# rslmtoasa/rslmtoasa

Measured on AMD Instinct MI355X. Metric: block-recursion throughput (H|psi> + A_n + B_n recursion levels, recursion.f90 recur_b), higher is better.
Workload: dtype f64

## Files before the change

### rslmtoasa_amd/csrc/kernels_spmm5.hpp

```cpp
#pragma once
#include <hip/hip_runtime.h>
#include <algorithm>
#include <type_traits>
#include <vector>
#include "kernels_valu.hpp"
#include "kernels_mfma.hpp"
#include "kernels_spmm4.hpp"

namespace rsrec {

#ifndef RSREC_S5_KSPLIT_PROBE
#define RSREC_S5_KSPLIT_PROBE 0
#endif
#ifndef RSREC_S5_PRIO
#define RSREC_S5_PRIO 0
#endif
#ifndef S5_WG_GROUPS
#define S5_WG_GROUPS 4
#endif
constexpr int S5_TRIPLE = 640;
constexpr int S5_TRIPLE_BYTES = S5_TRIPLE * 8;
constexpr int S5_HEAD_TRIPLES = 2;
constexpr int S5_HEAD_DOUBLES = 2 * S5_HEAD_TRIPLES * S5_TRIPLE;
constexpr int S5_MAXENT = 2 * S4_MAXSLOTS + 2;
constexpr int S5_ENTPAD = 8;

struct S5Desc { const double* a; const double* b; double sign; double diag; };

__device__ __forceinline__ double s5_desc_value(const S5Desc& D, int ro, int ri, int c ) {
    double v = D.sign * D.a[2 * (ro + 18 * ri) + c];
    if (D.b) v = v + D.b[2 * (ro + 18 * ri) + c];
    if (D.diag != 0.0 && ro == ri && c == 0) v = v + D.diag;
    return v;
}

__global__ __launch_bounds__(640) void k_s5_emit(const S5Desc* __restrict__ desc, const int* __restrict__ meta, int meta_stride, int nfs, int null_col, int ntr,
                                                 double* __restrict__ frag) {
    const int t = blockIdx.x, sig = blockIdx.y, st = blockIdx.z;
    const int* codes = meta + (size_t)st * meta_stride + 2;
    const S5Desc* D = desc + (size_t)st * nfs;
    const int e0 = threadIdx.x;
    const int K = e0 < 256 ? 0 : e0 < 512 ? 1 : 2;
    const int r = e0 - (K == 0 ? 0 : K == 1 ? 256 : 512);
    int q, l, e;
    if (K < 2) { q = r >> 7; l = (r & 127) >> 1; e = r & 1; } else { q = r >> 6; l = r & 63; e = 0; }
    const int k = l >> 4, rho = q == 0 ? (l & 15) : 16 + (l & 3);
    const int stq = rho >> 2, ll = rho & 3;
    int po = 0, mo = 0;
    bool row = true;
    if (stq < 4) { po = stq & 1; mo = 4 * (stq >> 1) + ll; } else if (ll < 2) { po = ll; mo = 8; } else row = false;
    const int o0 = 10 * t + (K == 0 ? 0 : K == 1 ? 4 : 8);
    const int o = K < 2 ? o0 + k : o0 + (k >> 1);
    const int pi = K < 2 ? e : (k & 1);
    double v = 0.0;
    if (row) {
        const int j = o / 9, code = codes[j], col = code & 255, flip = code >> 8;
        if (col != null_col && D[col].a) {
            const int so = sig, si = flip ? 1 - sig : sig, mi = o % 9;
            const int ro = 9 * so + mo, ri = 9 * si + mi;
            const double hr = s5_desc_value(D[col], ro, ri, 0), hi = s5_desc_value(D[col], ro, ri, 1);
            v = (po == pi) ? hr : (po == 0 ? -hi : hi);
        }
    }
    frag[(((size_t)st * 2 + sig) * ntr + t) * S5_TRIPLE + e0] = v;
}

struct Spmm5Operator {
    double* d_frag = nullptr;
    int* d_meta = nullptr;
    size_t frag_bytes = 0, meta_bytes = 0;
    S5Desc* d_desc = nullptr;
    size_t desc_bytes = 0;
    std::vector<signed char> sched_sig;
    int sched_dims[3] = {0, 0, 0};
    int sched_epoch = 0;
    int ntau = 0, nslots = 0, have_o = 0, ntr = 0, spin_mixing = 0;
    static constexpr int META = 2 + S5_MAXENT + S5_ENTPAD;
    struct Entry { const double* blk; int col; int flip; };
    struct Head { std::vector<double> blk; int flip = 0; bool valid = false; };
    std::vector<Head> head_main;
    std::vector<int> ksteps;
    std::vector<signed char> mixing;

    Spmm5Operator() = default;
    Spmm5Operator(const Spmm5Operator&) = delete;
    Spmm5Operator& operator=(const Spmm5Operator&) = delete;
    ~Spmm5Operator() { release(); }
    void release() {
        if (d_frag) (void)hipFree(d_frag);
        if (d_meta) (void)hipFree(d_meta);
        if (d_desc) (void)hipFree(d_desc);
        d_frag = nullptr; d_meta = nullptr; d_desc = nullptr; frag_bytes = meta_bytes = desc_bytes = 0;
        sched_sig.clear();
    }
    static bool decode20(int rho, int& part, int& m) {
        const int st = rho >> 2, l = rho & 3;
        if (st < 4) { part = st & 1; m = 4 * (st >> 1) + l; return true; }
        if (l < 2) { part = l; m = 8; return true; }
        return false;
    }
    static double hreal(const double* blk, int so, int po, int mo, int si, int pi, int mi) {
        const int ro = 9 * so + mo, ri = 9 * si + mi;
        const double hr = blk[2 * (ro + 18 * ri)], hi = blk[2 * (ro + 18 * ri) + 1];
        if (po == pi) return hr;
        return po == 0 ? -hi : hi;
    }
    static int steps_of(int nent) {
        const int n = 9 * nent, r = n % 10;
        return 3 * (n / 10) + (r == 0 ? 0 : r <= 4 ? 1 : r <= 8 ? 2 : 3);
    }
// ... 17 lines not shown
                    }
            }
        }
    }
    const char* make_schedule(int nslots_lat, int ntau_, int nset, const std::vector<signed char>& kind, std::vector<std::vector<std::pair<int, int>>>* sched_out) {
        if (nslots_lat + 1 > S4_MAXSLOTS) return "too many neighbour slots for the spmm5 kernel";
        const bool same = !sched_out && d_meta && sched_dims[0] == nslots_lat && sched_dims[1] == ntau_ && sched_dims[2] == nset && sched_sig == kind;
        if (same) return nullptr;
        ++sched_epoch;
        ntau = ntau_; nslots = nslots_lat; have_o = nset > 1 ? 1 : 0; spin_mixing = 0;
        const int nfs = nslots + 1, null_col = nslots + 1;
        std::vector<std::vector<std::pair<int, int>>> sched((size_t)nset * ntau);
        std::vector<int> meta((size_t)nset * ntau * META, 0);
        ksteps.assign((size_t)nset * ntau, 0);
        mixing = kind;
        int maxent = 0;
        for (int set = 0; set < nset; ++set)
            for (int tau = 0; tau < ntau; ++tau) {
                std::vector<std::pair<int, int>>& E = sched[(size_t)set * ntau + tau];
                const signed char* Kd = kind.data() + ((size_t)set * ntau + tau) * nfs;
                int* M = meta.data() + ((size_t)set * ntau + tau) * META;
                if (Kd[nslots] >= 0) {
                    E.push_back({nslots, 0});
                    E.push_back({Kd[nslots] == 1 ? nslots : -1, 1});
                    M[1] = 2;
                }
                for (int s = 0; s < nslots; ++s) {
                    if (Kd[s] < 0) continue;
                    E.push_back({s, 0});
                    if (Kd[s] == 1) { E.push_back({s, 1}); if (s > 0) spin_mixing = 1; }
                }
                M[0] = steps_of((int)E.size());
                ksteps[(size_t)set * ntau + tau] = 5 * (M[0] / 3) + 2 * (M[0] % 3);
                for (int j = 0; j < S5_MAXENT + S5_ENTPAD; ++j)
                    M[2 + j] = j < (int)E.size() ? ((E[j].first >= 0 ? E[j].first : null_col) | (E[j].second << 8)) : null_col;
                maxent = std::max(maxent, (int)E.size());
            }
        ntr = (9 * maxent + 9) / 10 + 1;
        const size_t need = (size_t)nset * ntau * 2 * ntr * S5_TRIPLE * sizeof(double), mneed = meta.size() * sizeof(int);
        if (need > frag_bytes) {
            if (d_frag) (void)hipFree(d_frag);
            d_frag = nullptr; frag_bytes = 0;
            if (hipMalloc(reinterpret_cast<void**>(&d_frag), need) != hipSuccess) return "hipMalloc of spmm5 operator fragments failed";
            frag_bytes = need;
        }
        if (mneed > meta_bytes) {
            if (d_meta) (void)hipFree(d_meta);
            d_meta = nullptr; meta_bytes = 0;
            if (hipMalloc(reinterpret_cast<void**>(&d_meta), mneed) != hipSuccess) return "hipMalloc of spmm5 schedule failed";
            meta_bytes = mneed;
        }
        if (hipMemcpy(d_meta, meta.data(), mneed, hipMemcpyHostToDevice) != hipSuccess) return "upload of spmm5 schedule failed";
        sched_sig = kind; sched_dims[0] = nslots_lat; sched_dims[1] = ntau_; sched_dims[2] = nset;
        if (sched_out) sched_out->swap(sched);
        return nullptr;
    }
    static std::vector<signed char> kinds_of(const std::vector<const double*>& blk) {
        std::vector<signed char> kind(blk.size(), -1);
        for (size_t q = 0; q < blk.size(); ++q)
            if (blk[q]) kind[q] = Spmm4Operator::pattern_of(blk[q]) == 0 ? 1 : 0;
        return kind;
    }
    const char* build_custom(int nslots_lat, int ntau_, int nset, const std::vector<const double*>& blk) {
        std::vector<std::vector<std::pair<int, int>>> sched;
        if (const char* msg = make_schedule(nslots_lat, ntau_, nset, kinds_of(blk), &sched)) return msg;
        const int nfs = nslots + 1;
        head_main.assign((size_t)nset * ntau, Head());
        const size_t per_sig = (size_t)ntr * S5_TRIPLE, per_set = (size_t)ntau * 2 * per_sig;
// ... 105 lines not shown
template <int NL, int NM>
__device__ __forceinline__ void s5_interleave() {
    constexpr int PER = NM / NL;
#pragma unroll
    for (int i = 0; i < NL; ++i) {
        __builtin_amdgcn_sched_group_barrier(0x20, 1, 0);
        __builtin_amdgcn_sched_group_barrier(0x8, PER, 0);
    }
    __builtin_amdgcn_sched_group_barrier(0x8, NM - PER * NL, 0);
}

template <int NL = 11>
__device__ __forceinline__ void s5_mfma(S5Acc& acc, const S5Pair& o) {
#pragma unroll
    for (int e = 0; e < 2; ++e)
#pragma unroll
        for (int t = 0; t < 9; ++t) {
            acc.m[t] = __builtin_amdgcn_mfma_f64_16x16x4f64(o.a[0][e], o.b[t][e], acc.m[t], 0, 0, 0);
            acc.r[t] = __builtin_amdgcn_mfma_f64_4x4x4f64(o.a[1][e], o.b[t][e], acc.r[t], 0, 0, 0);
        }
    s5_interleave<NL, 36>();
}
template <int NL = 11>
__device__ __forceinline__ void s5_mfma(S5Acc& acc, const S5Single& o) {
#pragma unroll
    for (int t = 0; t < 9; ++t) {
        acc.m[t] = __builtin_amdgcn_mfma_f64_16x16x4f64(o.a[0], o.b[t], acc.m[t], 0, 0, 0);
        acc.r[t] = __builtin_amdgcn_mfma_f64_4x4x4f64(o.a[1], o.b[t], acc.r[t], 0, 0, 0);
    }
    s5_interleave<NL, 18>();
}

template <int N> using S5C = std::integral_constant<int, N>;
#define S5_GLOBAL __attribute__((address_space(1)))
#define S5_CONST __attribute__((address_space(4)))
#define S5_LDS __attribute__((address_space(3)))
typedef const S5_GLOBAL char* s5_gp;

template <bool TWO, bool LDSA, bool OCT = false>
__device__ __forceinline__ void s5_run_stream(S5Acc& acc, const int* __restrict__ meta, const char* __restrict__ fr , const char* __restrict__ fr_head,
                                              const char* __restrict__ inb, const char* __restrict__ in2b,
                                              const int* __restrict__ nbr5 ,
                                              const int (&atom)[GROUP] , int rem_sel ,
                                              int ncol, int sig, int l4,
                                              unsigned lane_main, unsigned lane_z, unsigned lane_rem, unsigned lane_rem_z, unsigned lane16, unsigned lane8,
                                              const int (&tile_blk)[GROUP], int rem_blk , int kpart = 0) {
    int left = meta[0];
    int ebase = 0, tbase = 0;
    bool first = true;
#if RSREC_S5_KSPLIT_PROBE
    if (kpart == 0) left = min(left, 27);
    else { left -= 27; ebase = 10; tbase = 9; first = false; }
#endif
    if (left <= 0) return;
    const bool extras = TWO && meta[1] != 0;
    const S5_CONST int* codes = (const S5_CONST int*)(meta + 2);
    const S5_CONST int* nbr = (const S5_CONST int*)nbr5;
    S5Ent E0, E1;
    int raw[GROUP];
    int code_cur = codes[ebase], code_nxt = codes[ebase + 1];
    auto load_idx = [&](int col) {
#pragma unroll
        for (int t = 0; t < GROUP; ++t) raw[t] = nbr[(size_t)ncol * atom[t] + col];
    };
    load_idx(code_cur & 255);
    unsigned vlane_main = lane_main, vlane_z = lane_z, vlane16 = lane16, vlane8 = lane8;
    auto open_entry = [&](int j, S5Ent& E) {
        const unsigned so = 2592u * (unsigned)((code_cur >> 8) ? 1 - sig : sig);
#pragma unroll
        for (int t = 0; t < GROUP; ++t) E.off[t] = (unsigned)(OCT ? raw[t] + tile_blk[t] : raw[t]) * (BLD * 8u) + so;
        const int r01 = (rem_sel & 1) ? raw[1] : raw[0], r23 = (rem_sel & 1) ? raw[3] : raw[2], r45 = (rem_sel & 1) ? raw[5] : raw[4], r67 = (rem_sel & 1) ? raw[7] : raw[6];
        const int r03 = (rem_sel & 2) ? r23 : r01, r47 = (rem_sel & 2) ? r67 : r45;
        E.rem = (unsigned)(((rem_sel & 4) ? r47 : r03) + (OCT ? rem_blk : 0)) * (BLD * 8u) + so;
        code_cur = code_nxt;
        code_nxt = codes[j + 2];
        load_idx(code_cur & 255);
    };
    auto issue = [&](auto s2c, auto& o) {
        constexpr int S2 = decltype(s2c)::value, S = S2 % 27, wrap = S2 / 27;
        using I = S5St<S>;
        S5Ent& EA = (I::eA & 1) ? E1 : E0;
        S5Ent& EB = (I::eA & 1) ? E0 : E1;
        if constexpr (I::opens) open_entry(ebase + 10 * wrap + I::eOpen, (I::eOpen & 1) ? E1 : E0);
        const bool head = wrap == 0 && first && extras;
        const char* __restrict__ base = (TWO && S < 5 && head) ? in2b : inb;
        s5_gp fbg = nullptr;
        if constexpr (!LDSA) {
            const char* fb = ((TWO && I::T < S5_HEAD_TRIPLES && head && fr_head) ? fr_head + I::T * S5_TRIPLE_BYTES
                                                                                 : fr + (size_t)(tbase + 9 * wrap + I::T) * S5_TRIPLE_BYTES)
// ... 31 lines not shown
#pragma unroll
            for (int q = 0; q < 2; ++q) o.a[q] = *(const S5_LDS V*)(fl + lf + q * (I::K < 2 ? 1024 : 512));
        } else if constexpr (I::K < 2) {
#pragma unroll
            for (int q = 0; q < 2; ++q) o.a[q] = *(const S5_GLOBAL V*)(fbg + lf + q * 1024);
        } else {
#pragma unroll
            for (int q = 0; q < 2; ++q) o.a[q] = *(const S5_GLOBAL V*)(fbg + lf + q * 512);
        }
    };
    S5Pair X, Y;
    S5Single Z;
    issue(S5C<0>{}, X);
    issue(S5C<1>{}, Y);
#define S5_STEP(S, NEXT, CUR)                 \
    if (left > (S)) {                         \
        issue(S5C<(S) + 2>{}, NEXT);          \
        s5_mfma<LDSA ? 9 : 11>(acc, CUR);     \
        __builtin_amdgcn_sched_barrier(0);    \
    }
    for (;; left -= 27) {
        S5_STEP(0, Z, X) S5_STEP(1, X, Y) S5_STEP(2, Y, Z) S5_STEP(3, Z, X) S5_STEP(4, X, Y) S5_STEP(5, Y, Z)
        S5_STEP(6, Z, X) S5_STEP(7, X, Y) S5_STEP(8, Y, Z) S5_STEP(9, Z, X) S5_STEP(10, X, Y) S5_STEP(11, Y, Z)
        S5_STEP(12, Z, X) S5_STEP(13, X, Y) S5_STEP(14, Y, Z) S5_STEP(15, Z, X) S5_STEP(16, X, Y) S5_STEP(17, Y, Z)
        S5_STEP(18, Z, X) S5_STEP(19, X, Y) S5_STEP(20, Y, Z) S5_STEP(21, Z, X) S5_STEP(22, X, Y) S5_STEP(23, Y, Z)
        S5_STEP(24, Z, X) S5_STEP(25, X, Y) S5_STEP(26, Y, Z)
        if (left <= 27) break;
        ebase += 10; tbase += 9; first = false;
    }
#undef S5_STEP
}


template <int NT> struct S5PairN { s5_d2 b[NT]; s5_d2 a[2]; };
template <int NT> struct S5SingleN { double b[NT]; double a[2]; };
template <int NT> struct S5AccN { double4_t m[NT]; double r[NT]; };

template <int NT>
__device__ __forceinline__ void s5_mfma_n(S5AccN<NT>& acc, const S5PairN<NT>& o) {
#pragma unroll
    for (int e = 0; e < 2; ++e)
#pragma unroll
        for (int t = 0; t < NT; ++t) {
            acc.m[t] = __builtin_amdgcn_mfma_f64_16x16x4f64(o.a[0][e], o.b[t][e], acc.m[t], 0, 0, 0);
            acc.r[t] = __builtin_amdgcn_mfma_f64_4x4x4f64(o.a[1][e], o.b[t][e], acc.r[t], 0, 0, 0);
        }
    s5_interleave<NT, 4 * NT>();
}
template <int NT>
__device__ __forceinline__ void s5_mfma_n(S5AccN<NT>& acc, const S5SingleN<NT>& o) {
#pragma unroll
    for (int t = 0; t < NT; ++t) {
        acc.m[t] = __builtin_amdgcn_mfma_f64_16x16x4f64(o.a[0], o.b[t], acc.m[t], 0, 0, 0);
        acc.r[t] = __builtin_amdgcn_mfma_f64_4x4x4f64(o.a[1], o.b[t], acc.r[t], 0, 0, 0);
    }
    s5_interleave<NT, 2 * NT>();
}

struct S5EntN { unsigned off[3]; unsigned rem; };

template <bool TWO, int NMAIN, bool HASREM>
__device__ __forceinline__ void s5_run_stream_n(S5AccN<NMAIN + (HASREM ? 1 : 0)>& acc, const int* __restrict__ meta, const char* __restrict__ fr ,
                                                const char* __restrict__ inb, const char* __restrict__ in2b, const int* __restrict__ nbr5,
                                                const int (&atom)[NMAIN], const int (&ratom)[GROUP], int rem_sel, int ncol, int sig, int l4,
                                                unsigned lane_main, unsigned lane_z, unsigned lane_rem, unsigned lane_rem_z, unsigned lane16, unsigned lane8) {
    constexpr int NT = NMAIN + (HASREM ? 1 : 0);
// ... 68 lines not shown
        const S5_LDS char* fl = (const S5_LDS char*)fr + (unsigned)(tbase + 9 * wrap + I::T) * S5_TRIPLE_BYTES + (I::K == 0 ? 0 : I::K == 1 ? 2048 : 4096);
#pragma unroll
        for (int q = 0; q < 2; ++q) o.a[q] = *(const S5_LDS V*)(fl + lf + q * (I::K < 2 ? 1024 : 512));
    };
    S5PairN<NT> X0, Y0, X1, Y1;
    S5SingleN<NT> Z0, Z1;
    issue(S5C<0>{}, X0);
    issue(S5C<1>{}, Y0);
    issue(S5C<2>{}, Z0);
    issue(S5C<3>{}, X1);
    issue(S5C<4>{}, Y1);
#define S5_STEP(S, NEXT, CUR)                 \
    if (left > (S)) {                         \
        issue(S5C<(S) + 5>{}, NEXT);          \
        s5_mfma_n<NT>(acc, CUR);              \
        __builtin_amdgcn_sched_barrier(0);    \
    }
    for (;; left -= 54) {
        S5_STEP(0, Z1, X0) S5_STEP(1, X0, Y0) S5_STEP(2, Y0, Z0) S5_STEP(3, Z0, X1) S5_STEP(4, X1, Y1) S5_STEP(5, Y1, Z1)
        S5_STEP(6, Z1, X0) S5_STEP(7, X0, Y0) S5_STEP(8, Y0, Z0) S5_STEP(9, Z0, X1) S5_STEP(10, X1, Y1) S5_STEP(11, Y1, Z1)
        S5_STEP(12, Z1, X0) S5_STEP(13, X0, Y0) S5_STEP(14, Y0, Z0) S5_STEP(15, Z0, X1) S5_STEP(16, X1, Y1) S5_STEP(17, Y1, Z1)
        S5_STEP(18, Z1, X0) S5_STEP(19, X0, Y0) S5_STEP(20, Y0, Z0) S5_STEP(21, Z0, X1) S5_STEP(22, X1, Y1) S5_STEP(23, Y1, Z1)
        S5_STEP(24, Z1, X0) S5_STEP(25, X0, Y0) S5_STEP(26, Y0, Z0) S5_STEP(27, Z0, X1) S5_STEP(28, X1, Y1) S5_STEP(29, Y1, Z1)
        S5_STEP(30, Z1, X0) S5_STEP(31, X0, Y0) S5_STEP(32, Y0, Z0) S5_STEP(33, Z0, X1) S5_STEP(34, X1, Y1) S5_STEP(35, Y1, Z1)
        S5_STEP(36, Z1, X0) S5_STEP(37, X0, Y0) S5_STEP(38, Y0, Z0) S5_STEP(39, Z0, X1) S5_STEP(40, X1, Y1) S5_STEP(41, Y1, Z1)
        S5_STEP(42, Z1, X0) S5_STEP(43, X0, Y0) S5_STEP(44, Y0, Z0) S5_STEP(45, Z0, X1) S5_STEP(46, X1, Y1) S5_STEP(47, Y1, Z1)
        S5_STEP(48, Z1, X0) S5_STEP(49, X0, Y0) S5_STEP(50, Y0, Z0) S5_STEP(51, Z0, X1) S5_STEP(52, X1, Y1) S5_STEP(53, Y1, Z1)
        if (left <= 54) break;
        ebase += 20; tbase += 18; first = false;
    }
#undef S5_STEP
}

struct S5Epilogue { int kind = 0; const double* cur = nullptr; const double* old = nullptr; double a = 1.0, b = 0.0; };

struct S5Gram { double* out = nullptr; size_t cstride = 0; long min_groups = 0; };

template <bool TWO, bool LDSA, bool OCT = false, int NSP = 1, bool GRAM = false>
__global__ __launch_bounds__(NSP == 3 ? 768 : S5_WG_GROUPS * 128) void k_spmm5(SpmmDims D, const int* __restrict__ order_all, const int* __restrict__ cum,
                                               const int* __restrict__ nbr ,
                                               const int* __restrict__ izp, const double* __restrict__ frag, const int* __restrict__ meta, int ntr,
                                               const double* __restrict__ in_all, double* __restrict__ out_all,
                                               const double* __restrict__ in2_all = nullptr,
                                               const double* __restrict__ frag_head = nullptr ,
                                               int ntau = 0, int lds_tau = 0 ,
                                               int* __restrict__ queue = nullptr ,
                                               int spin_by_xcd = 1 ,
                                               S5Epilogue epi = S5Epilogue(), S5Gram gram = S5Gram()) {
    static_assert(!GRAM || (!TWO && !OCT && NSP == 1), "the Gram epilogue: one input, whole groups of atoms");
    extern __shared__ double s5_lds[];
    const int lane = threadIdx.x & 63;
    const int wave = __builtin_amdgcn_readfirstlane(threadIdx.x >> 6);
    const int sig = LDSA ? (int)((spin_by_xcd ? blockIdx.x : (blockIdx.x >> 3)) & 1) : wave / S5_WG_GROUPS, gslot = LDSA ? wave : wave % S5_WG_GROUPS;
#if RSREC_S5_PRIO
    if (wave >= (int)(blockDim.x >> 7)) __builtin_amdgcn_s_setprio(1);
#endif
    const int WGG = LDSA ? (int)(blockDim.x >> 6) : S5_WG_GROUPS;
    int bxl = blockIdx.x, gdxl = gridDim.x, run_lo = D.run_lo, run_hi = D.run_hi, qrun = 0;
    if (LDSA && D.nruns > 0) {
        const int row = spin_by_xcd ? 8 : 16, rowi = (int)blockIdx.x / row;
        int r = 0;
#pragma unroll
        for (int q = 1; q < 4; ++q) if (q < D.nruns && rowi >= D.run_row0[q]) r = q;
        lds_tau = D.run_tau[r]; run_lo = D.run_glo[r]; run_hi = D.run_ghi[r];
        bxl = (int)blockIdx.x - row * D.run_row0[r];
        gdxl = row * (D.run_row0[r + 1] - D.run_row0[r]);
        qrun = r;
    }
    if constexpr (LDSA) {
        const s5_d2* __restrict__ src = reinterpret_cast<const s5_d2*>(frag + ((size_t)lds_tau * 2 + sig) * ntr * S5_TRIPLE);
        s5_d2* dst = reinterpret_cast<s5_d2*>(s5_lds);
        const int n = ntr * (S5_TRIPLE / 2);
        constexpr int PER = (int)(160 * 1024 / 16 / (NSP == 3 ? 512 : S5_WG_GROUPS * 64));
        const int nthr = (int)blockDim.x;
        s5_d2 v[PER];
#pragma unroll
        for (int i = 0; i < PER; ++i) { const int e = threadIdx.x + i * nthr; if (e < n) v[i] = src[e]; }
#pragma unroll
        for (int i = 0; i < PER; ++i) { const int e = threadIdx.x + i * nthr; if (e < n) dst[e] = v[i]; }
        __syncthreads();
    }
    const int l15 = lane & 15, l4 = lane >> 4;
    const unsigned lane_main = 8u * (36 * l4 + 2 * l15), lane_z = 8u * (36 * (l4 >> 1) + 2 * l15 + (l4 & 1));
    const unsigned lane_rem = 8u * (36 * l4 + 32 + 2 * (l15 & 1)), lane_rem_z = 8u * (36 * (l4 >> 1) + 32 + 2 * (l15 & 1) + (l4 & 1));
    const unsigned lane16 = 16u * lane, lane8 = 8u * lane;
    const int ncol = D.nslots + 2;
#pragma unroll 1
    for (int chain = OCT ? GROUP * (int)blockIdx.y : (int)blockIdx.y; chain < D.nchains; chain += OCT ? GROUP * (int)gridDim.y : (int)gridDim.y) {
    const int count = cum[(chain / D.cpo) * D.nlev + D.level];
    int ngroups = count / GROUP;
    const bool fold = GRAM && gram.out != nullptr && epi.kind == 0 && s5_gram_folds(ngroups, gram.min_groups);
    const int ob = D.obase[(chain / D.cpo) * D.nlev + D.level];
    const int* __restrict__ order = order_all + (size_t)(chain / D.cpo) * D.ostride + ob;
    const bool on_full_list = D.sat_base > 0 && ob == D.sat_base;
    if constexpr (OCT) ngroups = D.nmax;
    else if (run_hi > 0) {
        if (!on_full_list) continue;
        order += (size_t)run_lo * GROUP;
        ngroups = run_hi - run_lo;
    }
    const bool skipping = D.nskip > 0 && on_full_list;
    const size_t vo = (size_t)chain * D.vstride;
    const char* __restrict__ inb = reinterpret_cast<const char*>(in_all + vo);
    const char* __restrict__ in2b = TWO ? reinterpret_cast<const char*>(in2_all + vo) : nullptr;
    double* __restrict__ out = out_all + vo;
    const int zero_block = D.kk;

    int g, gend, gstep, glo = 0;
    bool dynamic = false;
    {
        const int bx = bxl;
        const int need = (ngroups + WGG - 1) / WGG;
        if constexpr (!LDSA) {
            const int nbx = max(1, min((int)gridDim.x, need));
            if (bx >= nbx) continue;
            if (nbx < 8) { g = bx * WGG + gslot; gend = ngroups; gstep = nbx * WGG; }
            else {
                const int xcd = bx & 7, j = bx >> 3;
                const int per_xcd = (nbx >> 3) + ((xcd < (nbx & 7)) ? 1 : 0);
                const int chunk = (ngroups + 7) >> 3;
                const int lo = xcd * chunk;
                gend = min(ngroups, lo + chunk);
                g = lo + j * WGG + gslot;
                gstep = per_xcd * WGG;
// ... 127 lines not shown
        int atom[GROUP];
        int vatom[GROUP], tile_blk[GROUP];
        int my_rem_atom, rem_blk = 0;
        if constexpr (OCT) {
            const int a0 = g;
#pragma unroll
            for (int t = 0; t < GROUP; ++t) {
                const bool ok = a0 >= 0 && chain + t < D.nchains;
                atom[t] = ok ? a0 : zero_block;
                tile_blk[t] = ok ? t * (D.kk + 1) : 0;
                vatom[t] = ok ? a0 + t * (D.kk + 1) : zero_block;
            }
            const int tr = l15 >> 1;
            const bool okr = a0 >= 0 && chain + tr < D.nchains;
            rem_blk = okr ? tr * (D.kk + 1) : 0;
            my_rem_atom = okr ? a0 + tr * (D.kk + 1) : zero_block;
        } else {
#pragma unroll
            for (int t = 0; t < GROUP; ++t) { const int a = grp[t]; atom[t] = a >= 0 ? a : zero_block; vatom[t] = atom[t]; tile_blk[t] = 0; }
            my_rem_atom = grp[l15 >> 1];
            my_rem_atom = my_rem_atom >= 0 ? my_rem_atom : zero_block;
        }
        const int first = atom[0];
        if (!OCT && D.skip_pa && first < D.nmax) continue;
        const int tau = first < D.nmax ? first : D.nmax + izp[first];
        const int* __restrict__ M = meta + (size_t)tau * Spmm5Operator::META;
        const char* __restrict__ fr = LDSA ? reinterpret_cast<const char*>(s5_lds) : reinterpret_cast<const char*>(frag + ((size_t)tau * 2 + sig) * ntr * S5_TRIPLE);
        const char* __restrict__ fh = (TWO && frag_head) ? reinterpret_cast<const char*>(frag_head + ((size_t)chain * ntau + tau) * S5_HEAD_DOUBLES + (size_t)sig * S5_HEAD_TRIPLES * S5_TRIPLE) : nullptr;

        S5Acc acc;
#pragma unroll
        for (int t = 0; t < 9; ++t) { acc.m[t] = (double4_t){0, 0, 0, 0}; acc.r[t] = 0.0; }

        if constexpr (OCT) s5_run_stream<TWO, LDSA, true>(acc, M, fr, fh, inb, in2b, nbr, atom, l15 >> 1, ncol, sig, l4, lane_main, lane_z, lane_rem, lane_rem_z, lane16, lane8, tile_blk, rem_blk);
        else s5_run_stream<TWO, LDSA>(acc, M, fr, fh, inb, in2b, nbr, atom, l15 >> 1, ncol, sig, l4, lane_main, lane_z, lane_rem, lane_rem_z, lane16, lane8, tile_blk, rem_blk, kpart);
#if RSREC_S5_KSPLIT_PROBE
        if (kpart) continue;
#endif

        if constexpr (GRAM) if (fold) {
            unsigned gl;
            asm volatile("v_mbcnt_lo_u32_b32 %0, -1, 0\n\tv_mbcnt_hi_u32_b32 %0, -1, %0" : "=v"(gl));
            const int lane = (int)gl, l15 = lane & 15, l4 = lane >> 4;
            const double* __restrict__ ub = in_all + vo;
            double4_t gre = {0, 0, 0, 0}, gim = {0, 0, 0, 0};
            double sre[2] = {0.0, 0.0}, sim[2] = {0.0, 0.0}, kre[2] = {0.0, 0.0}, kim[2] = {0.0, 0.0};
            auto rem_coef = [&](s5_d2 u, double& cr, double& ci) {
                cr = l4 == 0 ? u[0] : (l4 == 1 ? u[1] : 0.0);
                ci = l4 == 0 ? -u[1] : (l4 == 1 ? u[0] : 0.0);
            };
            auto gram_tiles = [&](auto t0c, auto t1c) {
                constexpr int T0 = decltype(t0c)::value, T1 = decltype(t1c)::value, NT = T1 - T0;
                s5_d2 gu[NT][3], gs[NT][3][2];
#pragma unroll
                for (int i = 0; i < NT; ++i) {
                    const int t = T0 + i;
                    const double* ab = ub + (size_t)BLD * ((t < 8) ? vatom[t] : my_rem_atom) + 324 * sig;
#pragma unroll
                    for (int p = 0; p < 3; ++p) {
                        const int row = 36 * (p < 2 ? 4 * p + l4 : 8);
                        if (t < 8) gu[i][p] = *reinterpret_cast<const s5_d2*>(ab + row + 2 * l15);
#pragma unroll
                        for (int e = 0; e < 2; ++e) gs[i][p][e] = *reinterpret_cast<const s5_d2*>(ab + row + 32 + 2 * e);
                    }
                }
#pragma unroll
                for (int i = 0; i < NT; ++i) {
                    const int t = T0 + i;
                    const double x8 = acc.r[t];
                    if (t < 8) {
#pragma unroll
                        for (int p = 0; p < 2; ++p) {
                            gre = __builtin_amdgcn_mfma_f64_16x16x4f64(gu[i][p][0], acc.m[t][2 * p], gre, 0, 0, 0);
                            gre = __builtin_amdgcn_mfma_f64_16x16x4f64(gu[i][p][1], acc.m[t][2 * p + 1], gre, 0, 0, 0);
                            gim = __builtin_amdgcn_mfma_f64_16x16x4f64(-gu[i][p][1], acc.m[t][2 * p], gim, 0, 0, 0);
                            gim = __builtin_amdgcn_mfma_f64_16x16x4f64(gu[i][p][0], acc.m[t][2 * p + 1], gim, 0, 0, 0);
                        }
                        double cr, ci;
                        rem_coef(gu[i][2], cr, ci);
                        gre = __builtin_amdgcn_mfma_f64_16x16x4f64(cr, x8, gre, 0, 0, 0);
                        gim = __builtin_amdgcn_mfma_f64_16x16x4f64(ci, x8, gim, 0, 0, 0);
                    }
                    double (&are)[2] = (t < 8) ? sre : kre;
                    double (&aim)[2] = (t < 8) ? sim : kim;
#pragma unroll
                    for (int e = 0; e < 2; ++e) {
#pragma unroll
                        for (int p = 0; p < 2; ++p) {
                            const double ur = gs[i][p][e][0], ui = gs[i][p][e][1], tr = acc.m[t][2 * p], ti = acc.m[t][2 * p + 1];
                            are[e] = fma(ur, tr, are[e]); are[e] = fma(ui, ti, are[e]);
                            aim[e] = fma(ur, ti, aim[e]); aim[e] = fma(-ui, tr, aim[e]);
                        }
                        double cr, ci;
                        rem_coef(gs[i][2][e], cr, ci);
                        are[e] = fma(cr, x8, are[e]);
                        aim[e] = fma(ci, x8, aim[e]);
                    }
                }
            };
            gram_tiles(S5C<0>{}, S5C<2>{});
            __builtin_amdgcn_sched_barrier(0);
            gram_tiles(S5C<2>{}, S5C<4>{});
            __builtin_amdgcn_sched_barrier(0);
            gram_tiles(S5C<4>{}, S5C<6>{});
            __builtin_amdgcn_sched_barrier(0);
            gram_tiles(S5C<6>{}, S5C<8>{});
            __builtin_amdgcn_sched_barrier(0);
            gram_tiles(S5C<8>{}, S5C<9>{});
            __builtin_amdgcn_sched_barrier(0);
            auto sum_l4 = [&](double v) {
                double s = __shfl(v, l15);
                s += __shfl(v, l15 + 16); s += __shfl(v, l15 + 32); s += __shfl(v, l15 + 48);
                return s;
            };
            auto sum_atoms = [&](double v) {
                double s = __shfl(v, l15 & 1);
#pragma unroll
                for (int a = 1; a < GROUP; ++a) s += __shfl(v, 2 * a + (l15 & 1));
                return s;
            };
            double* gp = gram.out + (size_t)chain * gram.cstride + ((size_t)g * 2 + sig) * S5_GRAM_DOUBLES;
            s5_d2 v;
#pragma unroll
            for (int p = 0; p < 2; ++p) {
                v[0] = gre[2 * p]; v[1] = gre[2 * p + 1];
                *reinterpret_cast<s5_d2*>(gp + 4 * lane + 2 * p) = v;
                v[0] = gim[2 * p]; v[1] = gim[2 * p + 1];
                *reinterpret_cast<s5_d2*>(gp + 256 + 4 * lane + 2 * p) = v;
            }
#pragma unroll
            for (int e = 0; e < 2; ++e) {
                v[0] = sum_l4(sre[e]); v[1] = sum_l4(sim[e]);
                if (l4 == e) *reinterpret_cast<s5_d2*>(gp + 512 + 2 * (16 * e + l15)) = v;
                v[0] = sum_atoms(sum_l4(kre[e])); v[1] = sum_atoms(sum_l4(kim[e]));
                if (lane < 2) *reinterpret_cast<s5_d2*>(gp + 576 + 2 * (2 * e + lane)) = v;
            }
        }
        const int ekind = GRAM ? 0 : epi.kind;
        auto finish = [&](auto t0c, auto t1c) {
            constexpr int T0 = decltype(t0c)::value, T1 = decltype(t1c)::value, NT = T1 - T0;
            size_t eo[NT];
#pragma unroll
// ... 12 lines not shown
                    const double* zb = epi.old + vo;
#pragma unroll
                    for (int i = 0; i < NT; ++i) {
#pragma unroll
                        for (int p = 0; p < 2; ++p) ez[i][p] = *reinterpret_cast<const s5_d2*>(zb + eo[i] + 36 * (4 * p + l4));
                        ezr[i] = zb[eo[i] + 288 + (l4 & 1)];
                    }
                }
            }
#pragma unroll
            for (int i = 0; i < NT; ++i) {
                const int t = T0 + i;
                const int a = (t < 8) ? vatom[t] : my_rem_atom;
                double* ob = out + eo[i];
#pragma unroll
                for (int p = 0; p < 2; ++p) {
                    s5_d2 v; v[0] = acc.m[t][2 * p]; v[1] = acc.m[t][2 * p + 1];
                    if (ekind) {
                        v[0] = (v[0] - epi.b * ec[i][p][0]) / epi.a; v[1] = (v[1] - epi.b * ec[i][p][1]) / epi.a;
                        if (ekind == 2) { v[0] = v[0] * 2.0 - ez[i][p][0]; v[1] = v[1] * 2.0 - ez[i][p][1]; }
                    }
                    if (a != zero_block) *reinterpret_cast<s5_d2*>(ob + 36 * (4 * p + l4)) = v;
                }
                double r = acc.r[t];
                if (ekind) {
                    r = (r - epi.b * ecr[i]) / epi.a;
                    if (ekind == 2) r = r * 2.0 - ezr[i];
                }
                if (a != zero_block && l4 < 2) ob[288 + l4] = r;
            }
        };
        finish(S5C<0>{}, S5C<5>{});
        finish(S5C<5>{}, S5C<9>{});
    }
    }
}

}
```

### rslmtoasa_amd/csrc/rsrec.hip

```cpp
#include <hip/hip_runtime.h>
#include <hsa/hsa.h>
#include <hsa/hsa_ext_amd.h>
#include <dlfcn.h>
#include <algorithm>
#include <array>
#include <atomic>
#include <chrono>
#include <cmath>
#include <cstdarg>
#include <cstdio>
#include <cstdlib>
#include <cstring>
#include <memory>
#include <string>
#include <thread>
#include <tuple>
#include <vector>

#include "../../include/rsrec.h"
#include "kernels_valu.hpp"
#include "kernels_mfma.hpp"
#include "kernels_spmm4.hpp"
#include "kernels_spmm5.hpp"
#include "kernels_uscheme.hpp"
// ... 77 lines not shown
    DevBuf d_la_extra, d_rot;
    Spmm5Operator kubo_op[RSREC_KUBO_NOUT_MAX], kubo_op_b[RSREC_KUBO_NIN_MAX], kubo_hbulk;
    Spmm5Operator orb_plain;
    DevBuf d_green_in, d_green_out;
    DevBuf d_kubo[5];
    DevBuf d_cond[4];
    DevBuf d_ctens[2];
    DevBuf d_bsqrt, d_term, d_gim, d_ldos;
    DevBuf d_ops, d_spec;
    struct SpecImage { int nop = 0, nen = 0, n = 0, site_offset = 0, nsites_total = 0; } spec_res;
    DevBuf d_mint;
    void* pin = nullptr;
    size_t pin_bytes = 0;
    DevBuf d_frags, d_vec[6], d_partial, d_partial2, d_coefA, d_coefB, d_bmats, d_status, d_seed, d_seedcoef, d_mu, d_scal, d_zsqr;
    DevBuf d_fan, d_fan_tab, d_mpair;
    DevBuf d_bloch_geo, d_bloch_tab;
    long opt_batch = 0, opt_kernels = 0, opt_nblk = 0, opt_spmm5 = 2, opt_chain_fold = 1, opt_s5_cap = 0, opt_side = 1, opt_s5_lds = 1, opt_s5_queue = 1, opt_cheb_fused = 1;
    long opt_s5_waves = 8;
    long opt_sat_pct = 100;
    long opt_orth_oop = 1;
    long opt_s5_split = 0;
    long opt_s5_run_min = 0;
    long opt_s5_spin_xcd = 0;
    long opt_s5_octet = 8;
    long opt_s5_host_emit = 0;
    long opt_kubo_lchunk = 0;
    long opt_kubo_vbatch = 0;
    long opt_kubo_setgroup = 0;
    int n_kubo_left_chunks = 0;
    int kubo_diag_nvec = 0, kubo_diag_ll = 0;
    long opt_orth3 = 1;
    long opt_graph = 1;
    long opt_s5_gram_min = 256;
    int ham_hermitian = 0;
    std::vector<int> opp_slot;
    int opp_epoch = -1;
    DevBuf d_gram;
    double n_gram_folded = 0, n_gram_all = 0, n_gram_levels = 0;
    hipGraphExec_t graph_exec = nullptr;
    std::vector<uintptr_t> graph_key;
    bool capturing = false;
    double t_total_ms = 0, t_hop_ms = 0, t_rest_ms = 0, t_host_ms = 0;
    double t_rot_ms = 0;
    double n_hop_launch = 0, n_atom_steps = 0, n_block_mult = 0, n_hop_mfma_flop = 0;
    double n_req_flop = 0;
    int hop_fuses_a = 1;
    std::vector<hipEvent_t> ev_pool;
    size_t ev_used = 0;
    struct RegionEntry {
        std::vector<int> seeds;
        int nlev, napply, flags, epoch, ostride;
        double atom_steps, block_mults;
        DevBuf order, cum;
        std::vector<int> level_max;
        std::vector<int> hop_min, hop_max;
        std::vector<double> level_groups;
        std::vector<double> mult_hist;
        struct ClassRun { int tau, lo, hi; };
        std::vector<ClassRun> sat_runs;
        std::vector<int> level_sat;
        int sat_base = 0;
    };
    std::vector<std::unique_ptr<RegionEntry>> region_cache;
    int lattice_epoch = 0;
    const int* cur_order = nullptr;
    const int* cur_cum = nullptr;
// ... 9 lines not shown
    int comm_rank = 0, comm_nranks = 1;
    DevBuf d_comm;
    ~rsrec_handle();
};

namespace {

struct OptionEntry { const char* name; long rsrec_handle::*member; };
const OptionEntry OPTIONS[] = {
    {"batch", &rsrec_handle::opt_batch},
    {"kernels", &rsrec_handle::opt_kernels},
    {"nblk", &rsrec_handle::opt_nblk},
    {"spmm5", &rsrec_handle::opt_spmm5},
    {"chain_fold", &rsrec_handle::opt_chain_fold},
    {"s5_cap", &rsrec_handle::opt_s5_cap},
    {"s5_lds", &rsrec_handle::opt_s5_lds},
    {"s5_queue", &rsrec_handle::opt_s5_queue},
    {"cheb_fused", &rsrec_handle::opt_cheb_fused},
    {"side_stream", &rsrec_handle::opt_side},
    {"graph", &rsrec_handle::opt_graph},
    {"orth3", &rsrec_handle::opt_orth3},
    {"s5_waves", &rsrec_handle::opt_s5_waves},
    {"s5_split", &rsrec_handle::opt_s5_split},
    {"orth_oop", &rsrec_handle::opt_orth_oop},
    {"sat_pct", &rsrec_handle::opt_sat_pct},
    {"kubo_lchunk", &rsrec_handle::opt_kubo_lchunk},
    {"kubo_vbatch", &rsrec_handle::opt_kubo_vbatch},
    {"kubo_setgroup", &rsrec_handle::opt_kubo_setgroup},
    {"s5_host_emit", &rsrec_handle::opt_s5_host_emit},
    {"s5_octet", &rsrec_handle::opt_s5_octet},
    {"s5_spin_xcd", &rsrec_handle::opt_s5_spin_xcd},
    {"s5_run_min", &rsrec_handle::opt_s5_run_min},
    {"s5_gram_min", &rsrec_handle::opt_s5_gram_min},
};

int fail(rsrec_t* h, int code, const char* fmt, ...) {
    char buf[512];
    va_list ap;
    va_start(ap, fmt);
    vsnprintf(buf, sizeof buf, fmt, ap);
    va_end(ap);
    if (h) h->err = buf;
    return code;
}

#define HIPCK(h, call)                                                                                         \
    do {                                                                                                       \
        hipError_t e_ = (call);                                                                                \
        if (e_ != hipSuccess) return fail(h, RSREC_ERR_DEVICE, "%s failed: %s (%s:%d)", #call, hipGetErrorString(e_), __FILE__, __LINE__); \
    } while (0)

hipEvent_t next_event(rsrec_t* h) {
    static const bool off = getenv("RSREC_NO_EVENTS") != nullptr;
    if (off || h->capturing) return nullptr;
    if (h->ev_used == h->ev_pool.size()) {
        hipEvent_t e;
        if (hipEventCreate(&e) != hipSuccess) return nullptr;
        h->ev_pool.push_back(e);
    }
    hipEvent_t e = h->ev_pool[h->ev_used++];
    (void)hipEventRecord(e, h->stream);
    return e;
}

constexpr size_t PIN_BYTES = (size_t)8 << 20;
int pin_ready(rsrec_t* h) {
// ... 847 lines not shown
        dim3 g2(std::max(row, (grid.x + row - 1) / row * row), grid.y);
        int* queue = nullptr;
        const unsigned ncu = (unsigned)std::max(16, h->n_cu / 16 * 16);
        if ((h->opt_s5_queue == 1 && grid.x >= ncu) || h->opt_s5_queue >= 2) {
            if ((!h->capturing || h->d_s5queue.bytes >= (size_t)SD.nchains * 16 * sizeof(int)) &&
                h->d_s5queue.reserve((size_t)SD.nchains * 16 * sizeof(int)) == hipSuccess &&
                hipMemsetAsync(h->d_s5queue.p, 0, (size_t)SD.nchains * 16 * sizeof(int), h->stream) == hipSuccess) {
                queue = h->d_s5queue.as<int>();
                g2 = dim3(ncu, 1);
            }
        }
        const unsigned thr = (queue && h->opt_s5_waves == 4) ? S5_WG_GROUPS * 64 : S5_WG_GROUPS * 128;
        if (queue && h->opt_s5_split == 3) {
            const unsigned thr3 = 64u * (unsigned)std::min<long>(12, std::max<long>(8, h->opt_s5_waves));
            const size_t lds3 = std::min(lds_limit, lds_bytes + (size_t)S5_TRIPLE_BYTES);
            k_spmm5<TWO, true, false, 3><<<g2, thr3, lds3, h->stream>>>(SD, order, cum, h->d_nbr5.as<int>(), iz, op.frag_set(set), op.meta_set(set), op.ntr, in, out, in2, nullptr, ntau, one, queue, spin_by_xcd, epi);
        } else if constexpr (!TWO) {
            if (gram.out) k_spmm5<false, true, false, 1, true><<<g2, thr, lds_bytes, h->stream>>>(SD, order, cum, h->d_nbr5.as<int>(), iz, op.frag_set(set), op.meta_set(set), op.ntr, in, out, in2, nullptr, ntau, one, queue, spin_by_xcd, epi, gram);
            else k_spmm5<false, true><<<g2, thr, lds_bytes, h->stream>>>(SD, order, cum, h->d_nbr5.as<int>(), iz, op.frag_set(set), op.meta_set(set), op.ntr, in, out, in2, nullptr, ntau, one, queue, spin_by_xcd, epi);
        } else
        k_spmm5<TWO, true><<<g2, thr, lds_bytes, h->stream>>>(SD, order, cum, h->d_nbr5.as<int>(), iz, op.frag_set(set), op.meta_set(set), op.ntr, in, out, in2, nullptr, ntau, one, queue, spin_by_xcd, epi);
    } else if constexpr (!TWO) {
        if (gram.out) k_spmm5<false, false, false, 1, true><<<grid, S5_WG_GROUPS * 128, 0, h->stream>>>(SD, order, cum, h->d_nbr5.as<int>(), iz, op.frag_set(set), op.meta_set(set), op.ntr, in, out, in2, extra, ntau, 0, nullptr, 1, epi, gram);
        else k_spmm5<false, false><<<grid, S5_WG_GROUPS * 128, 0, h->stream>>>(SD, order, cum, h->d_nbr5.as<int>(), iz, op.frag_set(set), op.meta_set(set), op.ntr, in, out, in2, extra, ntau, 0, nullptr, 1, epi);
    } else
        k_spmm5<TWO, false><<<grid, S5_WG_GROUPS * 128, 0, h->stream>>>(SD, order, cum, h->d_nbr5.as<int>(), iz, op.frag_set(set), op.meta_set(set), op.ntr, in, out, in2, extra, ntau, 0, nullptr, 1, epi);
}

template <bool TWO>
void launch_s5(rsrec_t* h, dim3 grid, const SpmmDims& SD0, const int* order, const int* cum, const int* iz, const Spmm5Operator& op, int set,
               const double* in, double* out, const double* in2 = nullptr, const double* extra = nullptr, int ntau = 0, S5Epilogue epi = S5Epilogue(),
               S5Gram gram = S5Gram() ) {
    SpmmDims SD = SD0;
    const int one = op.single_class(set);
    const rsrec_handle::RegionEntry* E = h->cur_entry;
    const bool multi = one < 0 && h->opt_s5_lds >= 2 && !extra && E && E->sat_base > 0 && SD.cpo == 1 && SD.level >= 0 && SD.level < (int)E->level_sat.size() &&
                       E->level_sat[SD.level] > 0 && op.ntau == h->nmax + h->ntype && (grid.x >= (unsigned)std::max(16, h->n_cu / 16 * 16) || h->opt_s5_queue >= 2) && (size_t)op.ntr * S5_TRIPLE * sizeof(double) <= (s5_prepare(h), h->s5_lds_limit);
    bool octets = false, oct_aside = false;
    double pa_pairs = 0.0;
    if (h->cur_level_groups && SD.level >= 0 && (size_t)(SD.level + 1) * op.ntau <= h->cur_level_groups->size() && op.ntau == h->nmax + h->ntype)
        for (int t = 0; t < h->nmax; ++t) pa_pairs += (*h->cur_level_groups)[(size_t)SD.level * op.ntau + t];
    if (!multi && one < 0 && h->opt_s5_octet > 0 && h->nmax >= h->opt_s5_octet && !extra && E && SD.cpo == 1 && SD.nchains >= 2 && op.ntau == h->nmax + h->ntype &&
        2.0 * pa_pairs >= (double)h->nmax * SD.nchains && (double)GROUP * (double)(h->kk + 1) * BLD * 8.0 < 4294967296.0) {
        SpmmDims SO = SD;
        const dim3 go((unsigned)((h->nmax + S5_WG_GROUPS - 1) / S5_WG_GROUPS), (unsigned)((SD.nchains + GROUP - 1) / GROUP));
        hipStream_t so = h->stream;
        if (h->opt_side && !h->oct_stream && !h->capturing &&
            (hipStreamCreateWithFlags(&h->oct_stream, hipStreamNonBlocking) != hipSuccess || hipEventCreateWithFlags(&h->ev_oct_in, hipEventDisableTiming) != hipSuccess ||
             hipEventCreateWithFlags(&h->ev_oct_out, hipEventDisableTiming) != hipSuccess)) { h->oct_stream = nullptr; (void)hipGetLastError(); }
        if (h->opt_side && h->oct_stream && h->ev_oct_in && h->ev_oct_out && hipEventRecord(h->ev_oct_in, h->stream) == hipSuccess &&
            hipStreamWaitEvent(h->oct_stream, h->ev_oct_in, 0) == hipSuccess) { so = h->oct_stream; oct_aside = true; }
        k_spmm5<TWO, false, true><<<go, S5_WG_GROUPS * 128, 0, so>>>(SO, order, cum, h->d_nbr5.as<int>(), iz, op.frag_set(set), op.meta_set(set), op.ntr, in, out, in2, nullptr, ntau,
                                                                   0, nullptr, 1, epi);
        if (oct_aside) (void)hipEventRecord(h->ev_oct_out, h->oct_stream);
        const bool all_sat = E->sat_base > 0 && SD.level < (int)E->level_sat.size() && E->level_sat[SD.level] == SD.nchains && (int)E->sat_runs.size() >= h->nmax &&
                             E->sat_runs[0].tau == 0 && E->sat_runs[0].lo == 0 && E->sat_runs[h->nmax - 1].tau == h->nmax - 1 && E->sat_runs[h->nmax - 1].hi == h->nmax;
        if (all_sat) {
            SD.sat_base = E->sat_base; SD.run_lo = h->nmax; SD.run_hi = E->sat_runs.back().hi;
        } else SD.skip_pa = 1;
        octets = true;
        h->n_octet_launch++;
    }
    if (!multi) {
        launch_s5_one<TWO>(h, grid, SD, order, cum, iz, op, set, in, out, in2, extra, ntau, epi, one, gram);
        if (oct_aside) (void)hipStreamWaitEvent(h->stream, h->ev_oct_out, 0);
    } else {
// ... 2849 lines not shown
```

Before: 67190.

## Share Gram remainder strips via DPP broadcasts and add optional self-tail prefetch

The Gram epilogue now loads only its own remainder-row strip once per lane and uses DPP row-broadcast and pair-swap to hand each tile's strip values to the other lanes, replacing the per-tile global loads of those strips. The tiles are processed one at a time with a scheduling barrier after each. An opt-in mode (s5_tail_self, off by default) adds a second code table whose padding points at the self slot and issues touch loads on the remainder atom to warm the cache. The DPP path adds cross-lane moves and more register pressure from keeping all group tiles' gu values live.

```diff
diff --git a/rslmtoasa_amd/csrc/kernels_spmm5.hpp b/rslmtoasa_amd/csrc/kernels_spmm5.hpp
--- a/rslmtoasa_amd/csrc/kernels_spmm5.hpp
+++ b/rslmtoasa_amd/csrc/kernels_spmm5.hpp
@@ -24,6 +24,7 @@
 constexpr int S5_HEAD_DOUBLES = 2 * S5_HEAD_TRIPLES * S5_TRIPLE;
 constexpr int S5_MAXENT = 2 * S4_MAXSLOTS + 2;
 constexpr int S5_ENTPAD = 8;
+constexpr int S5_CODES = S5_MAXENT + S5_ENTPAD;
 
 struct S5Desc { const double* a; const double* b; double sign; double diag; };
 
@@ -75,7 +76,7 @@
     int sched_dims[3] = {0, 0, 0};
     int sched_epoch = 0;
     int ntau = 0, nslots = 0, have_o = 0, ntr = 0, spin_mixing = 0;
-    static constexpr int META = 2 + S5_MAXENT + S5_ENTPAD;
+    static constexpr int META = 2 + 2 * S5_CODES;
     struct Entry { const double* blk; int col; int flip; };
     struct Head { std::vector<double> blk; int flip = 0; bool valid = false; };
     std::vector<Head> head_main;
@@ -159,8 +160,11 @@
                 }
                 M[0] = steps_of((int)E.size());
                 ksteps[(size_t)set * ntau + tau] = 5 * (M[0] / 3) + 2 * (M[0] % 3);
-                for (int j = 0; j < S5_MAXENT + S5_ENTPAD; ++j)
-                    M[2 + j] = j < (int)E.size() ? ((E[j].first >= 0 ? E[j].first : null_col) | (E[j].second << 8)) : null_col;
+                for (int j = 0; j < S5_CODES; ++j) {
+                    const bool real = j < (int)E.size();
+                    M[2 + j] = real ? ((E[j].first >= 0 ? E[j].first : null_col) | (E[j].second << 8)) : null_col;
+                    M[2 + S5_CODES + j] = real ? M[2 + j] : nslots;
+                }
                 maxent = std::max(maxent, (int)E.size());
             }
         ntr = (9 * maxent + 9) / 10 + 1;
@@ -332,6 +336,18 @@
 }
 
 template <int N> using S5C = std::integral_constant<int, N>;
+template <int N>
+__device__ __forceinline__ double s5_row_bcast(double v) {
+    const int lo = __builtin_amdgcn_mov_dpp(__double2loint(v), 0x150 + N, 0xf, 0xf, false);
+    const int hi = __builtin_amdgcn_mov_dpp(__double2hiint(v), 0x150 + N, 0xf, 0xf, false);
+    return __hiloint2double(hi, lo);
+}
+__device__ __forceinline__ double s5_pair_swap(double v) {
+    const int lo = __builtin_amdgcn_mov_dpp(__double2loint(v), 0xB1, 0xf, 0xf, false);
+    const int hi = __builtin_amdgcn_mov_dpp(__double2hiint(v), 0xB1, 0xf, 0xf, false);
+    return __hiloint2double(hi, lo);
+}
+
 #define S5_GLOBAL __attribute__((address_space(1)))
 #define S5_CONST __attribute__((address_space(4)))
 #define S5_LDS __attribute__((address_space(3)))
@@ -344,7 +360,8 @@
                                               const int (&atom)[GROUP] , int rem_sel ,
                                               int ncol, int sig, int l4,
                                               unsigned lane_main, unsigned lane_z, unsigned lane_rem, unsigned lane_rem_z, unsigned lane16, unsigned lane8,
-                                              const int (&tile_blk)[GROUP], int rem_blk , int kpart = 0) {
+                                              const int (&tile_blk)[GROUP], int rem_blk , int kpart = 0,
+                                              bool tail_self = false ) {
     int left = meta[0];
     int ebase = 0, tbase = 0;
     bool first = true;
@@ -354,7 +371,7 @@
 #endif
     if (left <= 0) return;
     const bool extras = TWO && meta[1] != 0;
-    const S5_CONST int* codes = (const S5_CONST int*)(meta + 2);
+    const S5_CONST int* codes = (const S5_CONST int*)(meta + 2 + (tail_self ? S5_CODES : 0));
     const S5_CONST int* nbr = (const S5_CONST int*)nbr5;
     S5Ent E0, E1;
     int raw[GROUP];
@@ -452,6 +469,16 @@
 }
 
 
+__device__ __forceinline__ int s5_touch_tail(const double* __restrict__ ub, int rem_atom, int sig) {
+    unsigned gl;
+    asm volatile("v_mbcnt_lo_u32_b32 %0, -1, 0\n\tv_mbcnt_hi_u32_b32 %0, -1, %0" : "=v"(gl));
+    const int q = (int)(gl & 7);
+    const int blk = __shfl(rem_atom, (int)(gl >> 3) * 2);
+    const unsigned off = q < 7 ? 1728u + 128u * (unsigned)q : 2588u;
+    return *reinterpret_cast<const int*>(reinterpret_cast<const char*>(ub + (size_t)BLD * blk + 324 * sig) + off);
+}
+__device__ __forceinline__ void s5_touch_done(int v) { asm volatile("" ::"v"(v)); }
+
 template <int NT> struct S5PairN { s5_d2 b[NT]; s5_d2 a[2]; };
 template <int NT> struct S5SingleN { double b[NT]; double a[2]; };
 template <int NT> struct S5AccN { double4_t m[NT]; double r[NT]; };
@@ -586,7 +613,7 @@
 #undef S5_STEP
 }
 
-struct S5Epilogue { int kind = 0; const double* cur = nullptr; const double* old = nullptr; double a = 1.0, b = 0.0; };
+struct S5Epilogue { int kind = 0; const double* cur = nullptr; const double* old = nullptr; double a = 1.0, b = 0.0; int tail_self = 0; };
 
 struct S5Gram { double* out = nullptr; size_t cstride = 0; long min_groups = 0; };
 
@@ -644,6 +671,7 @@
     const int count = cum[(chain / D.cpo) * D.nlev + D.level];
     int ngroups = count / GROUP;
     const bool fold = GRAM && gram.out != nullptr && epi.kind == 0 && s5_gram_folds(ngroups, gram.min_groups);
+    const bool tail = epi.tail_self != 0 && (fold || (!GRAM && epi.kind != 0 && epi.cur == in_all));
     const int ob = D.obase[(chain / D.cpo) * D.nlev + D.level];
     const int* __restrict__ order = order_all + (size_t)(chain / D.cpo) * D.ostride + ob;
     const bool on_full_list = D.sat_base > 0 && ob == D.sat_base;
@@ -837,8 +865,10 @@
 #pragma unroll
         for (int t = 0; t < 9; ++t) { acc.m[t] = (double4_t){0, 0, 0, 0}; acc.r[t] = 0.0; }
 
-        if constexpr (OCT) s5_run_stream<TWO, LDSA, true>(acc, M, fr, fh, inb, in2b, nbr, atom, l15 >> 1, ncol, sig, l4, lane_main, lane_z, lane_rem, lane_rem_z, lane16, lane8, tile_blk, rem_blk);
-        else s5_run_stream<TWO, LDSA>(acc, M, fr, fh, inb, in2b, nbr, atom, l15 >> 1, ncol, sig, l4, lane_main, lane_z, lane_rem, lane_rem_z, lane16, lane8, tile_blk, rem_blk, kpart);
+        if constexpr (OCT) s5_run_stream<TWO, LDSA, true>(acc, M, fr, fh, inb, in2b, nbr, atom, l15 >> 1, ncol, sig, l4, lane_main, lane_z, lane_rem, lane_rem_z, lane16, lane8, tile_blk, rem_blk, 0, tail);
+        else s5_run_stream<TWO, LDSA>(acc, M, fr, fh, inb, in2b, nbr, atom, l15 >> 1, ncol, sig, l4, lane_main, lane_z, lane_rem, lane_rem_z, lane16, lane8, tile_blk, rem_blk, kpart, tail);
+        int touched = 0;
+        if constexpr (GRAM) if (tail) touched = s5_touch_tail(in_all + vo, my_rem_atom, sig);
 #if RSREC_S5_KSPLIT_PROBE
         if (kpart) continue;
 #endif
@@ -854,65 +884,72 @@
                 cr = l4 == 0 ? u[0] : (l4 == 1 ? u[1] : 0.0);
                 ci = l4 == 0 ? -u[1] : (l4 == 1 ? u[0] : 0.0);
             };
-            auto gram_tiles = [&](auto t0c, auto t1c) {
-                constexpr int T0 = decltype(t0c)::value, T1 = decltype(t1c)::value, NT = T1 - T0;
-                s5_d2 gu[NT][3], gs[NT][3][2];
-#pragma unroll
-                for (int i = 0; i < NT; ++i) {
-                    const int t = T0 + i;
-                    const double* ab = ub + (size_t)BLD * ((t < 8) ? vatom[t] : my_rem_atom) + 324 * sig;
-#pragma unroll
-                    for (int p = 0; p < 3; ++p) {
-                        const int row = 36 * (p < 2 ? 4 * p + l4 : 8);
-                        if (t < 8) gu[i][p] = *reinterpret_cast<const s5_d2*>(ab + row + 2 * l15);
-#pragma unroll
-                        for (int e = 0; e < 2; ++e) gs[i][p][e] = *reinterpret_cast<const s5_d2*>(ab + row + 32 + 2 * e);
+            s5_d2 rs[3], gu[GROUP][3];
+            {
+                const double* rb = ub + (size_t)BLD * my_rem_atom + 324 * sig + 32 + 2 * (l15 & 1);
+#pragma unroll
+                for (int p = 0; p < 3; ++p) rs[p] = *reinterpret_cast<const s5_d2*>(rb + 36 * (p < 2 ? 4 * p + l4 : 8));
+            }
+#pragma unroll
+            for (int t = 0; t < GROUP; ++t) {
+                const double* ab = ub + (size_t)BLD * vatom[t] + 324 * sig + 2 * l15;
+#pragma unroll
+                for (int p = 0; p < 3; ++p) gu[t][p] = *reinterpret_cast<const s5_d2*>(ab + 36 * (p < 2 ? 4 * p + l4 : 8));
+            }
+            const bool odd = (l15 & 1) != 0;
+            auto strip = [&](auto tc, auto ec, auto pc) {
+                constexpr int t = decltype(tc)::value, e = decltype(ec)::value, p = decltype(pc)::value;
+                s5_d2 g;
+                if constexpr (t < 8) { g[0] = s5_row_bcast<2 * t + e>(rs[p][0]); g[1] = s5_row_bcast<2 * t + e>(rs[p][1]); }
+                else {
+                    const double o0 = s5_pair_swap(rs[p][0]), o1 = s5_pair_swap(rs[p][1]);
+                    g[0] = odd == (e != 0) ? rs[p][0] : o0; g[1] = odd == (e != 0) ? rs[p][1] : o1;
+                }
+                return g;
+            };
+            auto gram_tile = [&](auto tc) {
+                constexpr int t = decltype(tc)::value;
+                const double x8 = acc.r[t];
+                if constexpr (t < 8) {
+#pragma unroll
+                    for (int p = 0; p < 2; ++p) {
+                        gre = __builtin_amdgcn_mfma_f64_16x16x4f64(gu[t][p][0], acc.m[t][2 * p], gre, 0, 0, 0);
+                        gre = __builtin_amdgcn_mfma_f64_16x16x4f64(gu[t][p][1], acc.m[t][2 * p + 1], gre, 0, 0, 0);
+                        gim = __builtin_amdgcn_mfma_f64_16x16x4f64(-gu[t][p][1], acc.m[t][2 * p], gim, 0, 0, 0);
+                        gim = __builtin_amdgcn_mfma_f64_16x16x4f64(gu[t][p][0], acc.m[t][2 * p + 1], gim, 0, 0, 0);
                     }
-                }
-#pragma unroll
-                for (int i = 0; i < NT; ++i) {
-                    const int t = T0 + i;
-                    const double x8 = acc.r[t];
-                    if (t < 8) {
-#pragma unroll
-                        for (int p = 0; p < 2; ++p) {
-                            gre = __builtin_amdgcn_mfma_f64_16x16x4f64(gu[i][p][0], acc.m[t][2 * p], gre, 0, 0, 0);
-                            gre = __builtin_amdgcn_mfma_f64_16x16x4f64(gu[i][p][1], acc.m[t][2 * p + 1], gre, 0, 0, 0);
-                            gim = __builtin_amdgcn_mfma_f64_16x16x4f64(-gu[i][p][1], acc.m[t][2 * p], gim, 0, 0, 0);
-                            gim = __builtin_amdgcn_mfma_f64_16x16x4f64(gu[i][p][0], acc.m[t][2 * p + 1], gim, 0, 0, 0);
-                        }
-                        double cr, ci;
-                        rem_coef(gu[i][2], cr, ci);
-                        gre = __builtin_amdgcn_mfma_f64_16x16x4f64(cr, x8, gre, 0, 0, 0);
-                        gim = __builtin_amdgcn_mfma_f64_16x16x4f64(ci, x8, gim, 0, 0, 0);
-                    }
-                    double (&are)[2] = (t < 8) ? sre : kre;
-                    double (&aim)[2] = (t < 8) ? sim : kim;
-#pragma unroll
-                    for (int e = 0; e < 2; ++e) {
-#pragma unroll
-                        for (int p = 0; p < 2; ++p) {
-                            const double ur = gs[i][p][e][0], ui = gs[i][p][e][1], tr = acc.m[t][2 * p], ti = acc.m[t][2 * p + 1];
-                            are[e] = fma(ur, tr, are[e]); are[e] = fma(ui, ti, are[e]);
-                            aim[e] = fma(ur, ti, aim[e]); aim[e] = fma(-ui, tr, aim[e]);
-                        }
-                        double cr, ci;
-                        rem_coef(gs[i][2][e], cr, ci);
-                        are[e] = fma(cr, x8, are[e]);
-                        aim[e] = fma(ci, x8, aim[e]);
-                    }
-                }
+                    double cr, ci;
+                    rem_coef(gu[t][2], cr, ci);
+                    gre = __builtin_amdgcn_mfma_f64_16x16x4f64(cr, x8, gre, 0, 0, 0);
+                    gim = __builtin_amdgcn_mfma_f64_16x16x4f64(ci, x8, gim, 0, 0, 0);
+                }
+                double (&are)[2] = (t < 8) ? sre : kre;
+                double (&aim)[2] = (t < 8) ? sim : kim;
+                auto column = [&](auto ec) {
+                    constexpr int e = decltype(ec)::value;
+                    auto kstep = [&](auto pc) {
+                        constexpr int p = decltype(pc)::value;
+                        const s5_d2 g = strip(tc, ec, pc);
+                        const double ur = g[0], ui = g[1], tr = acc.m[t][2 * p], ti = acc.m[t][2 * p + 1];
+                        are[e] = fma(ur, tr, are[e]); are[e] = fma(ui, ti, are[e]);
+                        aim[e] = fma(ur, ti, aim[e]); aim[e] = fma(-ui, tr, aim[e]);
+                    };
+                    kstep(S5C<0>{});
+                    kstep(S5C<1>{});
+                    double cr, ci;
+                    rem_coef(strip(tc, ec, S5C<2>{}), cr, ci);
+                    are[e] = fma(cr, x8, are[e]);
+                    aim[e] = fma(ci, x8, aim[e]);
+                };
+                column(S5C<0>{});
+                column(S5C<1>{});
+                __builtin_amdgcn_sched_barrier(0);
             };
-            gram_tiles(S5C<0>{}, S5C<2>{});
-            __builtin_amdgcn_sched_barrier(0);
-            gram_tiles(S5C<2>{}, S5C<4>{});
-            __builtin_amdgcn_sched_barrier(0);
-            gram_tiles(S5C<4>{}, S5C<6>{});
-            __builtin_amdgcn_sched_barrier(0);
-            gram_tiles(S5C<6>{}, S5C<8>{});
-            __builtin_amdgcn_sched_barrier(0);
-            gram_tiles(S5C<8>{}, S5C<9>{});
-            __builtin_amdgcn_sched_barrier(0);
+            gram_tile(S5C<0>{}); gram_tile(S5C<1>{}); gram_tile(S5C<2>{}); gram_tile(S5C<3>{});
+            gram_tile(S5C<4>{}); gram_tile(S5C<5>{}); gram_tile(S5C<6>{}); gram_tile(S5C<7>{});
+            gram_tile(S5C<8>{});
+#pragma unroll
+            for (int e = 0; e < 2; ++e) { asm volatile("" : "+v"(sre[e]), "+v"(sim[e]), "+v"(kre[e]), "+v"(kim[e])); }
             auto sum_l4 = [&](double v) {
                 double s = __shfl(v, l15);
                 s += __shfl(v, l15 + 16); s += __shfl(v, l15 + 32); s += __shfl(v, l15 + 48);
@@ -991,8 +1028,9 @@
         };
         finish(S5C<0>{}, S5C<5>{});
         finish(S5C<5>{}, S5C<9>{});
-    }
-    }
-}
-
-}
+        if constexpr (GRAM) s5_touch_done(touched);
+    }
+    }
+}
+
+}
diff --git a/rslmtoasa_amd/csrc/rsrec.hip b/rslmtoasa_amd/csrc/rsrec.hip
--- a/rslmtoasa_amd/csrc/rsrec.hip
+++ b/rslmtoasa_amd/csrc/rsrec.hip
@@ -133,6 +133,7 @@
     long opt_orth3 = 1;
     long opt_graph = 1;
     long opt_s5_gram_min = 256;
+    long opt_s5_tail_self = 0;
     int ham_hermitian = 0;
     std::vector<int> opp_slot;
     int opp_epoch = -1;
@@ -208,6 +209,7 @@
     {"s5_spin_xcd", &rsrec_handle::opt_s5_spin_xcd},
     {"s5_run_min", &rsrec_handle::opt_s5_run_min},
     {"s5_gram_min", &rsrec_handle::opt_s5_gram_min},
+    {"s5_tail_self", &rsrec_handle::opt_s5_tail_self},
 };
 
 int fail(rsrec_t* h, int code, const char* fmt, ...) {
@@ -1121,6 +1123,7 @@
                const double* in, double* out, const double* in2 = nullptr, const double* extra = nullptr, int ntau = 0, S5Epilogue epi = S5Epilogue(),
                S5Gram gram = S5Gram() ) {
     SpmmDims SD = SD0;
+    epi.tail_self = h->opt_s5_tail_self ? 1 : 0;
     const int one = op.single_class(set);
     const rsrec_handle::RegionEntry* E = h->cur_entry;
     const bool multi = one < 0 && h->opt_s5_lds >= 2 && !extra && E && E->sat_base > 0 && SD.cpo == 1 && SD.level >= 0 && SD.level < (int)E->level_sat.size() &&
```

After: 67730, median of 6. No clear change (+0.8%).
